# lowquark/uflow

Hardware: AMD Instinct MI355X
Metric: device-resident frame-CRC GiB/s (1500-B frames, validate: crc+valid per frame) (higher is better)
Workload: dtype u8

## Files before the change

### uflow_amd/csrc/frame_crc.hip

```cpp
#include "frame_crc_dev.hpp"

namespace ufc_dev {

struct RunAcc {
  uint32_t crc;
  uint32_t valid;
};

template <bool SEAL>
__device__ __forceinline__ void finish_set(const Lane& L, const KernelParams& p, const FrameDesc& d, const Chains& c,
                                           uint64_t set, int t, RunAcc& acc) {
  const uint32_t X0 = L.odd ? c.v2 : c.v0, X1 = L.odd ? c.v3 : c.v1;
  const uint32_t X2 = L.odd ? c.v0 : c.v2, X3 = L.odd ? c.v1 : c.v3;
  uint32_t lin = xor3(nib_mul<0>(L.lds, X0, L.K2), nib_mul<1>(L.lds, X1, L.K2), nib_mul<2>(L.lds, X2, L.K2)) ^
                 nib_mul<3>(L.lds, X3, L.K2);
  lin = row_xor16(lin);
  const uint32_t crc = ~lin;
  if (SEAL) {
    const uint64_t f = set * 4 + (uint64_t)L.grp;
    if (L.col == 15 && f < p.nframes && d.len >= 4u) {
      uint8_t* a = p.wbytes + d.start + d.n;
      if (((uintptr_t)a & 3u) == 0) {
        *as_global<g_u32w>((uint32_t*)a) = __builtin_bswap32(crc);
      } else {
// ... 132 lines not shown
    uint64_t r2;
    int t2;
    next_pos(r, tt, r2, t2);
    if (r2 != r) store_run<SEAL>(L, p, set_of(r, 0) * 4, acc);
  };

  FrameDesc d = desc_now(set_of(run, t));
  int parts = set_parts(d);
  while (set_slow(d, parts)) {
    slow_set<SEAL>(L, p, d, parts * JC, set_of(run, t), t, acc);
    after_set(run, t);
    next_pos(run, t, run, t);
    if (set_of(run, t) >= nsets) return;
    d = desc_now(set_of(run, t));
    parts = set_parts(d);
  }

  struct Cursor {
    uint64_t run;
    int t, part, parts;
    bool valid, slow;
    FrameDesc d;
  };
  uint64_t pre_a = 0, pre_b = 0;
  auto prefetch_offsets = [&](uint64_t r2, int t2) {
    if (VARLEN) {
      const uint64_t s2 = set_of(r2, t2);
      const uint64_t f = frame_index(s2 < nsets ? s2 : 0);
      pre_a = *as_global<g_u64>(p.offsets + f);
      pre_b = *as_global<g_u64>(p.offsets + f + 1);
    }
  };
  auto advance = [&](Cursor& c) {
    if (!c.valid || c.slow) {
      c.valid = false;
      return;
    }
    if (!SINGLE && c.part + 1 < c.parts) {
      c.part++;
      return;
    }
    uint64_t r2;
    int t2;
    next_pos(c.run, c.t, r2, t2);
    c.run = r2;
    c.t = t2;
    c.part = 0;
    if (set_of(r2, t2) >= nsets) {
      c.valid = false;
      return;
    }
    c.d = VARLEN ? make_desc(pre_a, pre_b - pre_a) : make_desc(frame_index(set_of(r2, t2)) * p.stride, p.frame_len);
    {
      uint64_t r3;
      int t3;
      next_pos(r2, t2, r3, t3);
      prefetch_offsets(r3, t3);
    }
    c.parts = set_parts(c.d);
    c.slow = set_slow(c.d, c.parts);
  };
  auto lane_base = [&](const Cursor& c) -> const uint8_t* { return p.bytes + c.d.start - c.d.pad + 16 * L.col; };

  Cursor C0{run, t, 0, parts, true, false, d};
  {
    uint64_t r2;
    int t2;
    next_pos(run, t, r2, t2);
    prefetch_offsets(r2, t2);
  }
  Cursor C1 = C0;
  advance(C1);
  Cursor C2 = C1;
  advance(C2);
  auto load_cursor = [&](const Cursor& c, ItemBuf<JC>& b) {
    const bool ok = c.valid && !c.slow;
    load_item<JC>(ok ? lane_base(c) : lane_base(C0), ok ? c.part : 0, b);
  };

  Chains c{0u, 0u, 0u, 0u, 0u};
  bool go_slow = false;
  uint64_t slow_run = 0;
  int slow_t = 0;
  auto step = [&](ItemBuf<JC>& cur, ItemBuf<JC>& nxt2) -> bool {
    {
      const bool ok = C2.valid && !C2.slow;
      const uint8_t* q = (ok ? lane_base(C2) : lane_base(C0)) + (int64_t)(ok ? C2.part : 0) * (JC * 256);
      const bool p0 = SINGLE || C0.part == 0;
      if (!p0) __builtin_assume(C0.part >= 1);
#pragma unroll
      for (int j = 0; j < JC; j++) {
        const u32x4 v = __builtin_nontemporal_load(as_global<g_u32x4>(q + 256 * j));
        nxt2.x[j] = make_uint4(v.x, v.y, v.z, v.w);
        __builtin_amdgcn_sched_barrier(0);
        if (p0)
          process_block<FREEZE>(L, C0.d, j, cur.x[j], c);
        else
          process_block<FREEZE>(L, C0.d, C0.part * JC + j, cur.x[j], c);
        __builtin_amdgcn_sched_barrier(0);
      }
    }
    if (SINGLE || C0.part + 1 == C0.parts) {
      finish_set<SEAL>(L, p, C0.d, c, set_of(C0.run, C0.t), C0.t, acc);
      after_set(C0.run, C0.t);
    }
    if (!C1.valid) return false;
    if (C1.slow) {
      go_slow = true;
      slow_run = C1.run;
      slow_t = C1.t;
      return false;
    }
    C0 = C1;
    C1 = C2;
    advance(C2);
    return true;
  };
  {
    ItemBuf<JC> X, Y, Z;
    load_cursor(C0, X);
    load_cursor(C1, Y);
    while (step(X, Z) && step(Y, X) && step(Z, Y)) {
    }
  }
  if (go_slow) {
    run = slow_run;
    t = slow_t;
    while (set_of(run, t) < nsets) {
      d = desc_now(set_of(run, t));
      parts = set_parts(d);
      slow_set<SEAL>(L, p, d, parts * JC, set_of(run, t), t, acc);
      after_set(run, t);
      next_pos(run, t, run, t);
    }
  }
}




constexpr int lean_loadv(int skip, int first, int mid, int last) { return skip | first << 1 | mid << 6 | last << 11; }
[[maybe_unused]] constexpr int kLoadvAllNT = lean_loadv(0, kFixAuxNT, kFixAuxNT, kFixAuxNT);
constexpr int kLoadvProduct = lean_loadv(0, 0, kFixAuxNT, kFixAuxNT);
template <int J, bool SEAL, int DEPTH, int SCHED, int WAVES, int LOADV = kLoadvProduct>
__global__ __launch_bounds__(WAVES * 64) void frame_crc_fixed_kernel(const KernelParams p) {
  static_assert(DEPTH >= 1 && DEPTH <= 3, "pipeline depth (4 spills at J = 6)");
  static_assert(DEPTH != 1 || SCHED != kSchedClaim, "depth 1: static schedules only");
  constexpr bool DYN = SCHED == kSchedClaim;
  constexpr bool ILV = SCHED == kSchedInterleave;
  constexpr uint32_t kInc = ILV ? (uint32_t)WAVES : 1u;
  __shared__ __attribute__((aligned(16))) char lds[kLdsBytes];
  const StageSet<WAVES * 64> sr = stage_load<WAVES * 64>(p);
  Lane L;
  init_lane(L, lds, p.G);

  const uint64_t stride = p.stride;
  const uint32_t len = (uint32_t)p.frame_len;
  const uint32_t n = len - 4u;
  const int pad = J * 256 - (int)len;
  const uint32_t nsets = (uint32_t)((p.nframes + 3) >> 2);
  const uint32_t nfull = (uint32_t)(p.nframes >> 2);
  const bool tail = (p.nframes & 3) != 0;
  const uint32_t wpb = WAVES;
  const uint32_t wid = __builtin_amdgcn_readfirstlane(threadIdx.x >> 6);
  const uint32_t w = blockIdx.x * wpb + wid;
  const uint32_t s_edge =
      p.front_ok ? 0u : (uint32_t)min(((uint64_t)pad + 4 * stride - 1) / (4 * stride), (uint64_t)nsets);
  const bool edge0 = s_edge == 1 && (p.nframes - 1) * stride + len >= 16;
  const uint32_t s_fast = edge0 ? 0u : s_edge;
  const uint32_t nfast = nfull - s_fast;
  uint32_t q_lo, q_end, q_cur, q_nx1, q_nx2;
  if (DYN || ILV) {
    q_lo = s_fast + (uint32_t)((uint64_t)nfast * blockIdx.x / gridDim.x);
    q_end = s_fast + (uint32_t)((uint64_t)nfast * (blockIdx.x + 1) / gridDim.x);
    q_cur = q_lo + wid;
    q_nx1 = q_lo + wpb + wid;
  } else {
    const uint32_t NW = gridDim.x * wpb;
    q_lo = s_fast + (uint32_t)((uint64_t)nfast * w / NW);
    q_end = s_fast + (uint32_t)((uint64_t)nfast * (w + 1) / NW);
    q_cur = q_lo;
    q_nx1 = q_lo + 1;
  }
  uint32_t* ctr = DYN ? p.ctr + blockIdx.x * kCtrWordsPerBlock : nullptr;
  auto claim_issue = [&]() -> uint32_t {
    uint32_t v = 0;
    if (L.lane == 0) v = __hip_atomic_fetch_add(ctr, 1u, __ATOMIC_RELAXED, __HIP_MEMORY_SCOPE_AGENT);
    return v;
  };
  auto claim_set = [&](uint32_t v) -> uint32_t {
    return q_lo + (DEPTH - 1) * wpb + __builtin_amdgcn_readfirstlane(v);
  };

  const int64_t lane_off = (int64_t)L.grp * (int64_t)stride + 16 * L.col - pad;
  uint32_t dm[4], pre[4];
#pragma unroll
  for (int b = 0; b < 4; b++) {
    const int o = 16 * L.col + 4 * b - pad;
    const uint32_t fz = fix_word(0u, o, L.G);
    const uint32_t f1 = fix_word(0xFFFFFFFFu, o, L.G);
    dm[b] = f1 & ~fz;
    pre[b] = fz;
  }
  uint32_t dm1, pre1;
  {
    const int o = 256 + 16 * L.col - pad;
    const uint32_t fz = fix_word(0u, o, L.G), f1 = fix_word(0xFFFFFFFFu, o, L.G);
    dm1 = f1 & ~fz;
    pre1 = fz;
  }
  const uint32_t tmask = (L.col == 15) ? 0u : 0xFFFFFFFFu;

  constexpr int RUNS = lean_runs(WAVES);
  uint32_t acc_crc = 0, acc_qv = 0;
  uint32_t hist_crc[RUNS], hist_qv[RUNS];
#pragma unroll
  for (int r = 0; r < RUNS; r++) hist_crc[r] = hist_qv[r] = 0;
  uint32_t t = 0, nhist = 0;
  auto write_trailer = [&](uint64_t f, uint32_t crc) {
    uint8_t* a = p.wbytes + f * stride + n;
    if (((uintptr_t)a & 3u) == 0) {
      *as_global<g_u32w>((uint32_t*)a) = __builtin_bswap32(crc);
    } else {
      g_u8w* wp = as_global<g_u8w>(a);
      wp[0] = (uint8_t)(crc >> 24);
      wp[1] = (uint8_t)(crc >> 16);
      wp[2] = (uint8_t)(crc >> 8);
      wp[3] = (uint8_t)crc;
    }
  };
  auto store_run = [&](int cnt, uint32_t crcs, uint32_t qv) {
    const uint64_t f = (uint64_t)(qv & 0x7FFFFFFFu) * 4 + (uint64_t)L.grp;
    if (L.col < cnt && f < p.nframes) {
      if (p.crc_out) *as_global<g_u32w>(p.crc_out + f) = crcs;
      if (!SEAL && p.valid_out) *as_global<g_u8w>(p.valid_out + f) = (uint8_t)(qv >> 31);
      if (SEAL) write_trailer(f, crcs);
    }
  };
  auto store_all = [&]() {
    if (t > 0) store_run((int)t, acc_crc, acc_qv);
#pragma unroll
    for (int r = 0; r < RUNS; r++)
      if ((uint32_t)r < nhist) store_run(kSetsPerRun, hist_crc[r], hist_qv[r]);
  };
  auto finish = [&](uint32_t q, const Chains& c, bool may_overflow) {
    const uint32_t crc = ~group_lin(L, c);
    const uint32_t tr = (uint32_t)__builtin_amdgcn_update_dpp(0, (int)c.tr, 0x15F, 0xF, 0xF, false);
    const uint32_t ok = (len >= 5u && __builtin_bswap32(tr) == crc) ? 1u : 0u;
    acc_crc = (L.col == (int)t) ? crc : acc_crc;
    acc_qv = (L.col == (int)t) ? (q | (ok << 31)) : acc_qv;
    if (++t == kSetsPerRun) {
      if (may_overflow && nhist == RUNS) {
        t = 0;
        store_all();
        __builtin_amdgcn_s_waitcnt(0x0F70);
        nhist = 0;
      }
#pragma unroll
      for (int r = RUNS - 1; r > 0; r--) {
        hist_crc[r] = hist_crc[r - 1];
        hist_qv[r] = hist_qv[r - 1];
      }
      hist_crc[0] = acc_crc;
      hist_qv[0] = acc_qv;
      nhist++;
      t = 0;
    }
  };
  auto compute_block = [&](uint32_t q, int j, uint4 x, Chains& c) {
    {
      if (j == J - 1) {
        c.tr = x.w;
        x.w &= tmask;
      }
      if (j == 0) {
        c.v0 = (x.x & dm[0]) | pre[0];
        c.v1 = (x.y & dm[1]) | pre[1];
        c.v2 = (x.z & dm[2]) | pre[2];
        c.v3 = (x.w & dm[3]) | pre[3];
      } else {
        if (j == 1) x.x = (x.x & dm1) | pre1;
        c.v0 = chain_step(L.lds, c.v0, L.K, x.x);
        c.v1 = chain_step(L.lds, c.v1, L.K, x.y);
        c.v2 = chain_step(L.lds, c.v2, L.K, x.z);
        c.v3 = chain_step(L.lds, c.v3, L.K, x.w);
      }
    }
  };
  auto compute = [&](uint32_t q, const ItemBuf<J>& b, Chains& c) {
#pragma unroll
    for (int j = 0; j < J; j++) compute_block(q, j, b.x[j], c);
  };
  const uint32_t voff = (uint32_t)(lane_off + 512);
  auto set_base = [&](uint32_t q) -> const uint8_t* {
    return p.bytes + (uint64_t)(q < q_end ? q : nfull - 1) * 4 * stride - 512;
  };
  auto load_edge0 = [&](ItemBuf<J>& b) {
    const int64_t room = (int64_t)min(p.nframes - 1, (uint64_t)3);
    const int64_t over = (int64_t)L.grp > room ? (int64_t)L.grp - room : 0;
    const int64_t off0 = lane_off - over * (int64_t)stride;
#pragma unroll
    for (int j = 0; j < J; j++) {
      const int64_t off = off0 + 256 * j;
      uint4 v = load_frame16<true>(p.bytes + (off < 0 ? 0 : off));
      if (off < 0) {
        const int64_t d = -off;
        uint64_t lo = (uint64_t)v.x | ((uint64_t)v.y << 32), hi = (uint64_t)v.z | ((uint64_t)v.w << 32);
        if (d >= 16) {
          lo = hi = 0;
        } else if (d >= 8) {
          hi = lo << (8 * (d - 8));
          lo = 0;
        } else {
          hi = (hi << (8 * d)) | (lo >> (64 - 8 * d));
          lo = lo << (8 * d);
        }
        v = make_uint4((uint32_t)lo, (uint32_t)(lo >> 32), (uint32_t)hi, (uint32_t)(hi >> 32));
      }
      b.x[j] = v;
    }
  };
  const uint32_t voff_b0 = ((LOADV & 1) && 16 * L.col + 16 <= pad - 4) ? kFixRecords : voff;
  auto load = [&](uint32_t q, ItemBuf<J>& b) {
    constexpr int kAuxFirst = (LOADV >> 1) & 31, kAuxMid = (LOADV >> 6) & 31, kAuxLast = (LOADV >> 11) & 31;
    const __amdgpu_buffer_rsrc_t rs =
        __builtin_amdgcn_make_buffer_rsrc((void*)set_base(q), 0, (int)kFixRecords, kFixRsrcWord3);
#pragma unroll
    for (int j = 0; j < J; j++) {
      const uint32_t o = (j == 0 ? voff_b0 : voff) + 256u * j;
      u32x4 v;
      if (j == 0)
        v = __builtin_amdgcn_raw_buffer_load_b128(rs, (int)o, 0, kAuxFirst);
      else if (j == J - 1)
        v = __builtin_amdgcn_raw_buffer_load_b128(rs, (int)o, 0, kAuxLast);
      else
        v = __builtin_amdgcn_raw_buffer_load_b128(rs, (int)o, 0, kAuxMid);
      b.x[j] = make_uint4(v.x, v.y, v.z, v.w);
    }
  };
  auto load_tail = [&](ItemBuf<J>& b) {
    const int64_t room = (int64_t)(p.nframes - 1 - 4 * (uint64_t)nfull);
    const int64_t over = (int64_t)L.grp > room ? (int64_t)L.grp - room : 0;
    load_set<J>(p.bytes + (uint64_t)nfull * 4 * stride - 512, voff - (uint32_t)(over * (int64_t)stride), b);
  };

  ItemBuf<J> A, B, C;
  uint32_t cX = 0, cY = 0, cZ = 0;
  if (DYN) {
    cY = claim_issue();
    cZ = claim_issue();
  }
  if (edge0 && q_cur == 0)
    load_edge0(A);
  else
    load(q_cur, A);
  if (DEPTH == 3) load(q_nx1, B);
  stage_store<WAVES * 64>(sr, lds);
  q_nx2 = (DEPTH == 3 && !DYN) ? q_cur + 2 * kInc : 0;

  if (w == 0 && s_fast > 0) {
#pragma unroll 1
    for (uint32_t e = 0; e < s_fast; e++) {
      FrameDesc d = make_desc(min((uint64_t)e * 4 + (uint64_t)L.grp, p.nframes - 1) * stride, len);
      Chains ce{0u, 0u, 0u, 0u, 0u};
#pragma unroll 1
      for (int blk = 0; blk < J; blk++) {
        uint32_t wv[4];
#pragma unroll
        for (int b = 0; b < 4; b++) {
          const int o = 256 * blk + 16 * L.col + 4 * b - d.pad;
          uint32_t a = 0;
#pragma unroll 1
          for (int k = 0; k < 4; k++) {
            const int ob = o + k;
            if (ob >= 0 && ob < (int)d.len) a |= (uint32_t)*as_global<g_u8>(p.bytes + d.start + (uint64_t)ob) << (8 * k);
          }
          wv[b] = a;
        }
        process_block<false>(L, d, blk, make_uint4(wv[0], wv[1], wv[2], wv[3]), ce);
      }
      const uint32_t crc = ~group_lin(L, ce);
      const uint32_t ok = (len >= 5u && __builtin_bswap32(ce.tr) == crc) ? 1u : 0u;
      const uint64_t f = (uint64_t)e * 4 + (uint64_t)L.grp;
      if (L.col == 15 && f < p.nframes) {
        if (p.crc_out) *as_global<g_u32w>(p.crc_out + f) = crc;
        if (!SEAL && p.valid_out) *as_global<g_u8w>(p.valid_out + f) = (uint8_t)ok;
        if (SEAL) write_trailer(f, crc);
      }
    }
    __builtin_amdgcn_s_waitcnt(0x0F70);
  }


  Chains c{0u, 0u, 0u, 0u, 0u};
  auto step = [&](ItemBuf<J>& cur, ItemBuf<J>& fill, uint32_t& c_issue, uint32_t& c_read) {
    uint32_t q_load;
    if (DYN) {
      q_load = claim_set(c_read);
      c_issue = claim_issue();
    } else {
      q_load = (DEPTH == 3) ? q_nx2 : q_nx1;
    }
    load(q_load, fill);
    __builtin_amdgcn_sched_barrier(0);
    if (q_cur < q_end) {
      compute(q_cur, cur, c);
      finish(q_cur, c, DYN);
    }
    __builtin_amdgcn_sched_barrier(0);
    if (DEPTH == 3) {
      q_cur = q_nx1;
      q_nx1 = q_load;
      q_nx2 = q_load + kInc;
    } else {
      q_cur = q_load;
      q_nx1 = q_load + kInc;
    }
  };
  if (DEPTH == 1) {
    while (q_cur < q_end) {
      compute(q_cur, A, c);
      finish(q_cur, c, false);
      q_cur += kInc;
      load(q_cur, A);
    }
  } else if (DEPTH == 2 && !DYN) {
    while (q_cur < q_end) {
      step(A, B, cX, cY);
      step(B, A, cY, cZ);
    }
  } else if (DEPTH == 2) {
    while (q_cur < q_end) {
      step(A, B, cX, cY);
      step(B, A, cY, cZ);
      step(A, B, cZ, cX);
      step(B, A, cX, cY);
      step(A, B, cY, cZ);
      step(B, A, cZ, cX);
    }
  } else {
    while (q_cur < q_end) {
      step(A, C, cX, cY);
      step(B, A, cY, cZ);
      step(C, B, cZ, cX);
    }
  }
  if (tail && blockIdx.x == gridDim.x - 1 && wid == wpb - 1) {
    ItemBuf<J> T;
    load_tail(T);
    compute(nfull, T, c);
    const uint32_t crc = ~group_lin(L, c);
    const uint32_t tr = (uint32_t)__builtin_amdgcn_update_dpp(0, (int)c.tr, 0x15F, 0xF, 0xF, false);
    const uint32_t ok = (len >= 5u && __builtin_bswap32(tr) == crc) ? 1u : 0u;
    const uint64_t f = (uint64_t)nfull * 4 + (uint64_t)L.grp;
    if (L.col == 0 && f < p.nframes) {
      if (p.crc_out) *as_global<g_u32w>(p.crc_out + f) = crc;
      if (!SEAL && p.valid_out) *as_global<g_u8w>(p.valid_out + f) = (uint8_t)ok;
      if (SEAL) write_trailer(f, crc);
    }
  }
  if (DYN) {
    store_all();
  } else {
    uint32_t blo = q_lo, bhi = q_end;
    if (!ILV) {
      const uint64_t NW = (uint64_t)gridDim.x * wpb;
      blo = s_fast + (uint32_t)((uint64_t)nfast * (blockIdx.x * wpb) / NW);
      bhi = s_fast + (uint32_t)((uint64_t)nfast * ((blockIdx.x + 1) * wpb) / NW);
    }
    const uint32_t nfr = 4 * (bhi - blo);
    uint32_t* lcrc = (uint32_t*)lds;
    uint8_t* lval = (uint8_t*)lds + 4 * nfr;
    __builtin_amdgcn_fence(__ATOMIC_RELEASE, "workgroup", "local");
    __builtin_amdgcn_s_barrier();
    __builtin_amdgcn_fence(__ATOMIC_ACQUIRE, "workgroup", "local");
    auto stage = [&](int cnt, uint32_t crcs, uint32_t qv) {
      if (L.col < cnt) {
        const uint32_t q = qv & 0x7FFFFFFFu;
        const uint32_t pos = (q - blo) * 4 + (uint32_t)L.grp;
        lcrc[pos] = crcs;
        lval[pos] = (uint8_t)(qv >> 31);
      }
    };
    if (t > 0) stage((int)t, acc_crc, acc_qv);
#pragma unroll
    for (int r = 0; r < RUNS; r++)
      if ((uint32_t)r < nhist) stage(kSetsPerRun, hist_crc[r], hist_qv[r]);
    __builtin_amdgcn_fence(__ATOMIC_RELEASE, "workgroup", "local");
    __builtin_amdgcn_s_barrier();
    __builtin_amdgcn_fence(__ATOMIC_ACQUIRE, "workgroup", "local");
    const uint64_t f0 = (uint64_t)blo * 4;
    if (p.crc_out)
      for (uint32_t i = threadIdx.x; i < nfr; i += WAVES * 64) *as_global<g_u32w>(p.crc_out + f0 + i) = lcrc[i];
    if (SEAL) {
      for (uint32_t i = threadIdx.x; i < nfr; i += WAVES * 64) {
        const uint32_t v = __builtin_bswap32(lcrc[i]);
        uint8_t* a = p.wbytes + (f0 + i) * stride + n;
        if (((uintptr_t)a & 3u) == 0) {
          __builtin_nontemporal_store(v, as_global<g_u32w>((uint32_t*)a));
        } else {
          g_u8w* wp = as_global<g_u8w>(a);
          __builtin_nontemporal_store((uint8_t)v, wp);
          __builtin_nontemporal_store((uint8_t)(v >> 8), wp + 1);
          __builtin_nontemporal_store((uint8_t)(v >> 16), wp + 2);
          __builtin_nontemporal_store((uint8_t)(v >> 24), wp + 3);
        }
      }
    }
    if (!SEAL && p.valid_out) {
      if ((((uintptr_t)(p.valid_out + f0)) & 3u) == 0) {
        for (uint32_t i = threadIdx.x; i < nfr / 4; i += WAVES * 64)
          *as_global<g_u32w>((uint32_t*)(p.valid_out + f0) + i) = ((const uint32_t*)lval)[i];
      } else {
        for (uint32_t i = threadIdx.x; i < nfr; i += WAVES * 64) *as_global<g_u8w>(p.valid_out + f0 + i) = lval[i];
      }
    }
  }

  if (DYN) {
    __builtin_amdgcn_s_waitcnt(0x0F70);
    uint32_t done = 0;
    if (L.lane == 0) done = __hip_atomic_fetch_add(ctr + 1, 1u, __ATOMIC_RELAXED, __HIP_MEMORY_SCOPE_AGENT);
    if (__builtin_amdgcn_readfirstlane(done) == wpb - 1 && L.lane == 0) {
      __hip_atomic_store(ctr, 0u, __ATOMIC_RELAXED, __HIP_MEMORY_SCOPE_AGENT);
      __hip_atomic_store(ctr + 1, 0u, __ATOMIC_RELAXED, __HIP_MEMORY_SCOPE_AGENT);
    }
  }
}

#define UFC_INST_FIXED(J)                                                                                  \
  template __global__ void frame_crc_fixed_kernel<J, false, 2, kSchedInterleave, 8>(const KernelParams); \
  template __global__ void frame_crc_fixed_kernel<J, true, 2, kSchedInterleave, 8>(const KernelParams);
UFC_INST_FIXED(1) UFC_INST_FIXED(2) UFC_INST_FIXED(3) UFC_INST_FIXED(4) UFC_INST_FIXED(5) UFC_INST_FIXED(6)


const void* fixed_kernel_symbol(int J, bool seal, int depth, int sched, int waves) {
  if (depth == 2 && sched == kSchedInterleave && waves == 8) {
    switch (J) {
#define UFC_PICK_FIXED(JJ)                                                                          \
  case JJ:                                                                                          \
    return seal ? (const void*)frame_crc_fixed_kernel<JJ, true, 2, kSchedInterleave, 8>          \
                : (const void*)frame_crc_fixed_kernel<JJ, false, 2, kSchedInterleave, 8>;
      UFC_PICK_FIXED(1) UFC_PICK_FIXED(2) UFC_PICK_FIXED(3) UFC_PICK_FIXED(4) UFC_PICK_FIXED(5) UFC_PICK_FIXED(6)
#undef UFC_PICK_FIXED
      default: return nullptr;
    }
  }
  return nullptr;
}

#define UFC_INST_MODES(JC)                                                                          \
  template __global__ void frame_crc_kernel<JC, 0>(const KernelParams);                             \
  template __global__ void frame_crc_kernel<JC, kModeSeal>(const KernelParams);                     \
  template __global__ void frame_crc_kernel<JC, kModeFreeze>(const KernelParams);                   \
  template __global__ void frame_crc_kernel<JC, kModeFreeze | kModeSeal>(const KernelParams);       \
  template __global__ void frame_crc_kernel<JC, kModeVarlen>(const KernelParams);                   \
  template __global__ void frame_crc_kernel<JC, kModeVarlen | kModeSeal>(const KernelParams);

#define UFC_CONFIGS(X) X(1) X(2) X(3) X(4) X(5) X(6)

UFC_CONFIGS(UFC_INST_MODES)


const void* kernel_symbol(int jc, int mode) {
#define UFC_PICK(JC)                                                                                   \
  if (jc == JC) {                                                                                      \
    switch (mode) {                                                                                    \
      case 0: return (const void*)frame_crc_kernel<JC, 0>;                                            \
      case kModeSeal: return (const void*)frame_crc_kernel<JC, kModeSeal>;                            \
      case kModeFreeze: return (const void*)frame_crc_kernel<JC, kModeFreeze>;                        \
      case kModeFreeze | kModeSeal: return (const void*)frame_crc_kernel<JC, kModeFreeze | kModeSeal>; \
      case kModeVarlen: return (const void*)frame_crc_kernel<JC, kModeVarlen>;                        \
      case kModeVarlen | kModeSeal: return (const void*)frame_crc_kernel<JC, kModeVarlen | kModeSeal>; \
      default: break;                                                                                  \
    }                                                                                                  \
  }
  UFC_CONFIGS(UFC_PICK)
#undef UFC_PICK
  return nullptr;
}

bool config_available(int jc) { return jc >= 1 && jc <= 6; }

namespace {
__global__ __launch_bounds__(256) void seal_scatter_kernel(uint8_t* bytes, uint64_t stride, uint64_t n_off,
                                                           uint64_t nframes, const uint32_t* crc) {
  for (uint64_t i = (uint64_t)blockIdx.x * 256 + threadIdx.x; i < nframes; i += (uint64_t)gridDim.x * 256) {
    const uint32_t v = __builtin_bswap32(crc[i]);
    uint8_t* a = bytes + i * stride + n_off;
    if (((uintptr_t)a & 3u) == 0) {
      __builtin_nontemporal_store(v, (uint32_t*)a);
    } else {
      __builtin_nontemporal_store((uint8_t)v, a);
      __builtin_nontemporal_store((uint8_t)(v >> 8), a + 1);
      __builtin_nontemporal_store((uint8_t)(v >> 16), a + 2);
      __builtin_nontemporal_store((uint8_t)(v >> 24), a + 3);
    }
  }
}
}

int seal_scatter(uint8_t* bytes, uint64_t stride, uint64_t frame_len, uint64_t nframes, const uint32_t* crc,
                 void* stream) {
  if (nframes == 0) return 0;
  const uint64_t blocks = std::min<uint64_t>((nframes + 255) / 256, 1u << 20);
  hipLaunchKernelGGL(seal_scatter_kernel, dim3((unsigned)blocks), dim3(256), 0, (hipStream_t)stream, bytes, stride,
                     frame_len - 4, nframes, crc);
  return (int)hipGetLastError();
}

}
```

### uflow_amd/csrc/frame_crc_kernels.hpp

```cpp
#pragma once
#include <cstdint>

namespace ufc_dev {

constexpr int kModeVarlen = 1;
constexpr int kModeSeal = 2;
constexpr int kModeFreeze = 4;

constexpr int kBlockThreads = 1024;
constexpr int kLdsBytes = 131072 + 32768;

struct KernelParams {
  const uint8_t* bytes;
  uint8_t* wbytes;
  const uint64_t* offsets;
  uint64_t stride;
  uint64_t frame_len;
  uint64_t nframes;
  uint32_t* crc_out;
  uint8_t* valid_out;
  const uint32_t* chain_tab;
  const uint32_t* nib_img;
  uint32_t G;
  uint32_t* ctr;
  uint32_t front_ok;
  uint32_t* defer_list;
  uint32_t* defer_counts;
};

const void* kernel_symbol(int jc, int mode);
bool config_available(int jc);
constexpr int kLeanDepthDefault = 2;
constexpr int kLeanRuns = 8;
constexpr int lean_runs(int waves) { return waves == 8 ? 32 : kLeanRuns; }
constexpr int kLeanWavesDefault = 8;
constexpr int kSchedRange = 0;
constexpr int kSchedClaim = 1;
constexpr int kSchedInterleave = 2;
constexpr int kLeanSchedDefault = kSchedInterleave;
const void* fixed_kernel_symbol(int J, bool seal, int depth, int sched, int waves);
constexpr int kRunFrames = 64;
const void* varlen8_kernel_symbol(bool seal, bool pairs);
int varlen8_waves();
const void* long8_kernel_symbol(bool seal, bool pairs);
int slots_to_pairs(const uint32_t* d_lens, uint64_t stride, uint64_t n, uint64_t* d_pairs, void* stream);
int seal_scatter(uint8_t* bytes, uint64_t stride, uint64_t frame_len, uint64_t nframes, const uint32_t* crc,
                 void* stream);
int read_stream(const uint8_t* bytes, uint64_t nbytes, uint32_t* sink, int ncu, void* stream);
constexpr int kCtrWordsPerBlock = 32;

}
```

### uflow_amd/csrc/ufc_api.cpp

```cpp
#include <hip/hip_runtime.h>

#include <algorithm>
#include <atomic>
#include <cstdio>
#include <cstdlib>
#include <cstring>
#include <mutex>
#include <new>
#include <vector>

#include "../../include/uflow_frame_codec.h"
#include "../../include/uflow_frame_crc.h"
#include "crc_math.hpp"
#include "frame_build.hpp"
#include "frame_crc_kernels.hpp"
#include "frame_pack.hpp"
#include "frame_parse.hpp"
#include "frame_queue.hpp"
#include "frame_window.hpp"
#include "flush_ctl.hpp"
#include "packet_emit.hpp"
#include "packet_receive.hpp"
#include "resend.hpp"
#include "route.hpp"
#include "send_rate.hpp"
#include "ufc_internal.hpp"

struct ufc_ctx {
  int device = -1;
  int ncu = 0;
  uint32_t* d_chain = nullptr;
  uint32_t* d_nib = nullptr;
  uint32_t* d_chain128 = nullptr;
  uint32_t* d_nib32 = nullptr;
  uint32_t G = 0;
  int last_hip_error = 0;
  std::atomic<int> stalled_comms{0};
  uint8_t* d_stage = nullptr;
  size_t d_stage_cap = 0;
  uint64_t* d_off = nullptr;
  size_t d_off_cap = 0;
  uint32_t* d_crc = nullptr;
  uint8_t* d_valid = nullptr;
  size_t d_out_cap = 0;
  uint64_t* h_off_pinned = nullptr;
  hipStream_t streams[2] = {nullptr, nullptr};
  uint32_t* d_ctr = nullptr;
  std::atomic<uint32_t> ctr_seq{0};
  int opt[UFC_OPT_COUNT_] = {};
  struct Scratch {
    int kind;
    hipStream_t stream;
    void* p;
    size_t cap;
  };
  std::mutex scratch_mu;
  std::vector<Scratch> scratch;
};

constexpr uint32_t kCtrSlots = 64;

namespace {

enum ScratchKind {
  kScratchParse = 0,
  kScratchAsyncSlots = 2,
  kScratchSealCrc = 3,
  kScratchDeferList = 4,
  kScratchDeferCounts = 5,
  kScratchBuild = 6,
  kScratchPack = 7,
  kScratchEmit = 8,
  kScratchReceive = 9,
  kScratchWindow = 10,
  kScratchFlushAcks = 11,
  kScratchFlushSync = 12,
  kScratchRoute = 13
};

hipError_t stream_scratch(ufc_ctx* ctx, int kind, hipStream_t stream, size_t need, void** out, bool* fresh = nullptr) {
  if (fresh) *fresh = false;
  std::lock_guard<std::mutex> lk(ctx->scratch_mu);
  ufc_ctx::Scratch* sc = nullptr;
  for (auto& x : ctx->scratch)
    if (x.kind == kind && x.stream == stream) sc = &x;
  if (!sc) {
    ctx->scratch.push_back({kind, stream, nullptr, 0});
    sc = &ctx->scratch.back();
  }
  if (sc->cap < need) {
    hipError_t e;
    if (sc->p) {
      if ((e = hipStreamSynchronize(stream)) != hipSuccess) return e;
      (void)hipFree(sc->p);
      sc->p = nullptr;
      sc->cap = 0;
    }
    if ((e = hipMalloc(&sc->p, need)) != hipSuccess) return e;
    sc->cap = need;
    if (fresh) *fresh = true;
  }
  *out = sc->p;
  return hipSuccess;
}

struct DeviceGuard {
  int prev = -1;
  explicit DeviceGuard(int dev) {
    if (hipGetDevice(&prev) != hipSuccess) prev = -1;
    if (prev != dev) (void)hipSetDevice(dev);
  }
  ~DeviceGuard() {
    int cur = -1;
    if (prev >= 0 && hipGetDevice(&cur) == hipSuccess && cur != prev) (void)hipSetDevice(prev);
  }
};

int hip_fail(ufc_ctx* ctx, hipError_t e) {
  if (ctx) ctx->last_hip_error = (int)e;
  return UFC_ERR_HIP;
}

struct Config {
  int jc;
};

int launch(ufc_ctx* ctx, Config cfg, int mode, ufc_dev::KernelParams& kp, hipStream_t stream) {
  const void* fn = ufc_dev::kernel_symbol(cfg.jc, mode);
  if (!fn) return UFC_ERR_INVALID_ARG;
  const uint64_t nsets = (kp.nframes + 3) / 4;
  const uint64_t nruns = (nsets + 15) / 16;
  const uint64_t waves_per_block = ufc_dev::kBlockThreads / 64;
  uint64_t blocks = (nruns + waves_per_block - 1) / waves_per_block;
  if (blocks > (uint64_t)ctx->ncu) blocks = (uint64_t)ctx->ncu;
  if (blocks < 1) blocks = 1;
  kp.chain_tab = ctx->d_chain;
  kp.nib_img = ctx->d_nib;
  kp.G = ctx->G;
  void* args[] = {&kp};
  hipError_t e = hipLaunchKernel(fn, dim3((unsigned)blocks), dim3(ufc_dev::kBlockThreads), args, 0, stream);
  if (e != hipSuccess) return hip_fail(ctx, e);
  return UFC_OK;
}

int lean_fixed_blocks(const ufc_ctx* ctx, uint64_t frame_len, uint64_t stride, uint64_t n) {
  if (frame_len < 4) return 0;
  const uint64_t J = (frame_len + 4 + 255) / 256;
  if (J > 6 || stride >= (1ull << 28)) return 0;
  const uint64_t pad = 256 * J - frame_len;
  const uint64_t s_edge = (pad + 4 * stride - 1) / (4 * stride);
  if (n / 4 <= s_edge) return 0;
  if (ctx->opt[UFC_OPT_FIXED_KERNEL] == UFC_FIXED_GENERIC || ctx->opt[UFC_OPT_GENERIC_JC] != 0) return 0;
  return (int)J;
}

int launch_lean_fixed(ufc_ctx* ctx, int J, bool seal, ufc_dev::KernelParams& kp, hipStream_t stream,
                      bool front_ok = false) {
  const int depth = ufc_dev::kLeanDepthDefault, waves = ufc_dev::kLeanWavesDefault;
  const int sched = ufc_dev::kLeanSchedDefault;
  const void* fn = ufc_dev::fixed_kernel_symbol(J, seal, depth, sched, waves);
  if (!fn) return UFC_ERR_INVALID_ARG;
  kp.chain_tab = ctx->d_chain;
  kp.nib_img = ctx->d_nib;
  kp.G = ctx->G;
  const uint64_t waves_per_block = (uint64_t)waves;
  const uint64_t chunk = (uint64_t)ctx->ncu * waves_per_block * (16 * ufc_dev::lean_runs(waves) - 1) * 4;
  const uint64_t total = kp.nframes;
  for (uint64_t f0 = 0, step = 0; f0 < total; f0 += step) {
    ufc_dev::KernelParams c = kp;
    c.nframes = std::min(chunk, total - f0);
    if (total - f0 - c.nframes > 0 && total - f0 - c.nframes < 4) c.nframes -= 4;
    step = c.nframes;
    c.bytes = kp.bytes + f0 * kp.stride;
    if (kp.wbytes) c.wbytes = kp.wbytes + f0 * kp.stride;
    if (kp.crc_out) c.crc_out = kp.crc_out + f0;
    if (kp.valid_out) c.valid_out = kp.valid_out + f0;
    c.front_ok = (f0 > 0 || front_ok) ? 1u : 0u;
    const uint32_t slot = ctx->ctr_seq.fetch_add(1) % kCtrSlots;
    c.ctr = ctx->d_ctr + (size_t)slot * ctx->ncu * ufc_dev::kCtrWordsPerBlock;
    const uint64_t nsets = (c.nframes + 3) / 4;
    uint64_t blocks = (nsets + waves_per_block - 1) / waves_per_block;
    if (blocks > (uint64_t)ctx->ncu) blocks = (uint64_t)ctx->ncu;
    if (blocks < 1) blocks = 1;
    void* args[] = {&c};
    hipError_t e = hipLaunchKernel(fn, dim3((unsigned)blocks), dim3((unsigned)(waves * 64)), args, 0, stream);
    if (e != hipSuccess) return hip_fail(ctx, e);
  }
  return UFC_OK;
}


int launch_varlen8(ufc_ctx* ctx, bool seal, bool pairs, ufc_dev::KernelParams& kp, hipStream_t stream) {
  const void* fn = ufc_dev::varlen8_kernel_symbol(seal, pairs);
  const void* fn_long = ufc_dev::long8_kernel_symbol(seal, pairs);
  if (!fn || !fn_long) return UFC_ERR_INVALID_ARG;
  const int waves = ufc_dev::varlen8_waves();
  kp.chain_tab = ctx->d_chain128;
  kp.nib_img = ctx->d_nib32;
  kp.G = ctx->G;
  const uint64_t chunk = (uint64_t)1 << 29;
  const uint64_t total = kp.nframes;
  void* list = nullptr;
  void* counts = nullptr;
  bool fresh = false;
  hipError_t e;
  const uint64_t nmax = std::min(chunk, total);
  if ((e = stream_scratch(ctx, kScratchDeferList, stream, (size_t)(nmax + 64) * 4, &list)) != hipSuccess ||
      (e = stream_scratch(ctx, kScratchDeferCounts, stream, (size_t)ctx->ncu * 4, &counts, &fresh)) != hipSuccess)
    return hip_fail(ctx, e);
  if (fresh && (e = hipMemsetAsync(counts, 0, (size_t)ctx->ncu * 4, stream)) != hipSuccess) return hip_fail(ctx, e);
  for (uint64_t f0 = 0; f0 < total; f0 += chunk) {
    ufc_dev::KernelParams c = kp;
    c.nframes = std::min(chunk, total - f0);
    c.offsets = kp.offsets + (pairs ? 2 * f0 : f0);
    if (kp.crc_out) c.crc_out = kp.crc_out + f0;
    if (kp.valid_out) c.valid_out = kp.valid_out + f0;
    c.defer_list = (uint32_t*)list;
    c.defer_counts = (uint32_t*)counts;
    const uint64_t nruns = (c.nframes + 63) / 64;
    uint64_t blocks = (nruns + waves - 1) / waves;
    if (blocks > (uint64_t)ctx->ncu) blocks = (uint64_t)ctx->ncu;
    if (blocks < 1) blocks = 1;
    void* args[] = {&c};
    if ((e = hipLaunchKernel(fn, dim3((unsigned)blocks), dim3((unsigned)(waves * 64)), args, 0, stream)) != hipSuccess)
      return hip_fail(ctx, e);
    uint32_t nb = (uint32_t)blocks;
    void* args_long[] = {&c, &nb};
    if ((e = hipLaunchKernel(fn_long, dim3((unsigned)blocks), dim3((unsigned)(waves * 64)), args_long, 0, stream)) !=
        hipSuccess)
      return hip_fail(ctx, e);
  }
  return UFC_OK;
}

Config fixed_config(const ufc_ctx* ctx, uint64_t frame_len, int* freeze) {
  const uint64_t n = frame_len >= 4 ? frame_len - 4 : frame_len;
  const uint64_t J = (n + 8 + 255) / 256;
  Config c;
  const int jc = ctx->opt[UFC_OPT_GENERIC_JC];
  c.jc = ufc_dev::config_available(jc) ? jc : (J <= 6 ? (int)J : 6);
  *freeze = ((uint64_t)c.jc == J) ? 0 : ufc_dev::kModeFreeze;
  return c;
}

Config varlen_config(const ufc_ctx* ctx) {
  const int jc = ctx->opt[UFC_OPT_GENERIC_JC];
  return Config{ufc_dev::config_available(jc) ? jc : 3};
}

int launch_varlen_any(ufc_ctx* ctx, bool seal, bool pairs, ufc_dev::KernelParams& kp, hipStream_t stream) {
  if (ctx->opt[UFC_OPT_VARLEN_KERNEL] == UFC_VARLEN_GENERIC && !pairs)
    return launch(ctx, varlen_config(ctx), ufc_dev::kModeVarlen | (seal ? ufc_dev::kModeSeal : 0), kp, stream);
  return launch_varlen8(ctx, seal, pairs, kp, stream);
}

using ufc_internal::kMaxFrameLen;

hipError_t grow_staging(ufc_ctx* ctx, size_t stage_bytes, size_t off_entries, size_t out_frames) {
  hipError_t e;
  if (ctx->d_stage_cap < stage_bytes) {
    if (ctx->d_stage) (void)hipFree(ctx->d_stage);
    ctx->d_stage = nullptr;
    ctx->d_stage_cap = 0;
    if ((e = hipMalloc(&ctx->d_stage, stage_bytes)) != hipSuccess) return e;
    ctx->d_stage_cap = stage_bytes;
  }
  if (ctx->d_off_cap < off_entries) {
    if (ctx->d_off) (void)hipFree(ctx->d_off);
    if (ctx->h_off_pinned) (void)hipHostFree(ctx->h_off_pinned);
    ctx->d_off = nullptr;
    ctx->h_off_pinned = nullptr;
    ctx->d_off_cap = 0;
    if ((e = hipMalloc(&ctx->d_off, off_entries * 8)) != hipSuccess) return e;
    if ((e = hipHostMalloc(&ctx->h_off_pinned, off_entries * 8, hipHostMallocDefault)) != hipSuccess) return e;
    ctx->d_off_cap = off_entries;
  }
  if (ctx->d_out_cap < out_frames) {
    if (ctx->d_crc) (void)hipFree(ctx->d_crc);
    if (ctx->d_valid) (void)hipFree(ctx->d_valid);
    ctx->d_crc = nullptr;
    ctx->d_valid = nullptr;
    ctx->d_out_cap = 0;
    if ((e = hipMalloc(&ctx->d_crc, out_frames * 4)) != hipSuccess) return e;
    if ((e = hipMalloc(&ctx->d_valid, out_frames)) != hipSuccess) return e;
    ctx->d_out_cap = out_frames;
  }
  return hipSuccess;
}

}

hipError_t ufc_dev::ScratchSource::get(size_t bytes, char** out) const {
  return stream_scratch(ctx, kind, stream, bytes, (void**)out);
}

extern "C" {

uint32_t ufc_crc32_compute(const uint8_t* data, size_t len) {
  if (!data) return 0;
  return ufc::host_extend(0u, data, len);
}

uint32_t ufc_crc32_extend(uint32_t initial_crc, const uint8_t* data, size_t len) {
  if (!data) return initial_crc;
  return ufc::host_extend(initial_crc, data, len);
}

int ufc_frame_validate(const uint8_t* frame, size_t len) {
  if (!frame || len < 5) return 0;
  const uint32_t c = ufc::host_extend(0u, frame, len - 4);
  const uint8_t* t = frame + len - 4;
  const uint32_t rx = ((uint32_t)t[0] << 24) | ((uint32_t)t[1] << 16) | ((uint32_t)t[2] << 8) | (uint32_t)t[3];
  return c == rx ? 1 : 0;
}

int ufc_frame_seal(uint8_t* frame, size_t len) {
  if (!frame || len < 4) return UFC_ERR_INVALID_ARG;
  const uint32_t c = ufc::host_extend(0u, frame, len - 4);
  uint8_t* t = frame + len - 4;
  t[0] = (uint8_t)(c >> 24);
  t[1] = (uint8_t)(c >> 16);
  t[2] = (uint8_t)(c >> 8);
  t[3] = (uint8_t)c;
  return UFC_OK;
}

int ufc_device_count(void) {
  int n = 0;
  if (hipGetDeviceCount(&n) != hipSuccess) return 0;
  return n;
}

const char* ufc_error_string(int code) {
  switch (code) {
    case UFC_OK: return "ok";
    case UFC_ERR_INVALID_ARG: return "invalid argument";
// ... 777 lines not shown
```

Baseline: 6120.

## Precompute lean partition geometry on host and issue first loads before LDS init

Moves the per-block work-range and edge computation (64-bit divides) into a host-side helper passed through kernel params as quotient/remainder. The first frame-set loads, plus the next one in the depth-2 static schedule, are issued before lane/LDS initialization. The old per-lane edge0 gather path is replaced by a clamped buffer load with an in-register shift fix. The depth-2 loop is peeled so the first set is computed outside the ping-pong loop. This targets kernel prologue latency, at the cost of a reordered params struct and new edge-case handling.

After: 6109. No clear change (-0.2%).

```diff
diff --git a/uflow_amd/csrc/frame_crc.hip b/uflow_amd/csrc/frame_crc.hip
--- a/uflow_amd/csrc/frame_crc.hip
+++ b/uflow_amd/csrc/frame_crc.hip
@@ -308,33 +308,32 @@
   __shared__ __attribute__((aligned(16))) char lds[kLdsBytes];
   const StageSet<WAVES * 64> sr = stage_load<WAVES * 64>(p);
   Lane L;
-  init_lane(L, lds, p.G);
+  L.lane = threadIdx.x & 63;
+  L.col = L.lane & 15;
+  L.grp = L.lane >> 4;
 
   const uint64_t stride = p.stride;
   const uint32_t len = (uint32_t)p.frame_len;
   const uint32_t n = len - 4u;
   const int pad = J * 256 - (int)len;
-  const uint32_t nsets = (uint32_t)((p.nframes + 3) >> 2);
   const uint32_t nfull = (uint32_t)(p.nframes >> 2);
   const bool tail = (p.nframes & 3) != 0;
   const uint32_t wpb = WAVES;
   const uint32_t wid = __builtin_amdgcn_readfirstlane(threadIdx.x >> 6);
   const uint32_t w = blockIdx.x * wpb + wid;
-  const uint32_t s_edge =
-      p.front_ok ? 0u : (uint32_t)min(((uint64_t)pad + 4 * stride - 1) / (4 * stride), (uint64_t)nsets);
-  const bool edge0 = s_edge == 1 && (p.nframes - 1) * stride + len >= 16;
-  const uint32_t s_fast = edge0 ? 0u : s_edge;
-  const uint32_t nfast = nfull - s_fast;
+  const bool front_ok = (p.lean_flags & kLeanFrontOk) != 0, edge0 = (p.lean_flags & kLeanEdge0) != 0;
+  const uint32_t s_fast = p.s_fast;
+  const uint32_t b_lo = lean_range_lo(s_fast, p.rq, p.rr, blockIdx.x);
+  const uint32_t b_end = lean_range_lo(s_fast, p.rq, p.rr, blockIdx.x + 1);
   uint32_t q_lo, q_end, q_cur, q_nx1, q_nx2;
   if (DYN || ILV) {
-    q_lo = s_fast + (uint32_t)((uint64_t)nfast * blockIdx.x / gridDim.x);
-    q_end = s_fast + (uint32_t)((uint64_t)nfast * (blockIdx.x + 1) / gridDim.x);
+    q_lo = b_lo;
+    q_end = b_end;
     q_cur = q_lo + wid;
     q_nx1 = q_lo + wpb + wid;
   } else {
-    const uint32_t NW = gridDim.x * wpb;
-    q_lo = s_fast + (uint32_t)((uint64_t)nfast * w / NW);
-    q_end = s_fast + (uint32_t)((uint64_t)nfast * (w + 1) / NW);
+    q_lo = b_lo + (uint32_t)((uint64_t)(b_end - b_lo) * wid / wpb);
+    q_end = b_lo + (uint32_t)((uint64_t)(b_end - b_lo) * (wid + 1) / wpb);
     q_cur = q_lo;
     q_nx1 = q_lo + 1;
   }
@@ -348,7 +347,72 @@
     return q_lo + (DEPTH - 1) * wpb + __builtin_amdgcn_readfirstlane(v);
   };
 
-  const int64_t lane_off = (int64_t)L.grp * (int64_t)stride + 16 * L.col - pad;
+  const int32_t lane_off = (int32_t)((uint32_t)L.grp * (uint32_t)stride) + 16 * L.col - pad;
+  const uint32_t voff = (uint32_t)(lane_off + 512);
+  auto set_base = [&](uint32_t q) -> const uint8_t* {
+    return p.bytes + (uint64_t)(q < q_end ? q : nfull - 1) * 4 * stride - 512;
+  };
+  const uint32_t voff_b0 = ((LOADV & 1) && 16 * L.col + 16 <= pad - 4) ? kFixRecords : voff;
+  constexpr int kAuxFirst = (LOADV >> 1) & 31, kAuxMid = (LOADV >> 6) & 31, kAuxLast = (LOADV >> 11) & 31;
+  auto load_block = [&](__amdgpu_buffer_rsrc_t rs, int j, uint32_t o) -> uint4 {
+    u32x4 v;
+    if (j == 0)
+      v = __builtin_amdgcn_raw_buffer_load_b128(rs, (int)o, 0, kAuxFirst);
+    else if (j == J - 1)
+      v = __builtin_amdgcn_raw_buffer_load_b128(rs, (int)o, 0, kAuxLast);
+    else
+      v = __builtin_amdgcn_raw_buffer_load_b128(rs, (int)o, 0, kAuxMid);
+    return make_uint4(v.x, v.y, v.z, v.w);
+  };
+  auto load = [&](uint32_t q, ItemBuf<J>& b) {
+    const __amdgpu_buffer_rsrc_t rs =
+        __builtin_amdgcn_make_buffer_rsrc((void*)set_base(q), 0, (int)kFixRecords, kFixRsrcWord3);
+#pragma unroll
+    for (int j = 0; j < J; j++) b.x[j] = load_block(rs, j, (j == 0 ? voff_b0 : voff) + 256u * j);
+  };
+  auto load_first = [&](uint32_t q, ItemBuf<J>& b) {
+    const uint64_t boff = (uint64_t)(q < q_end ? q : nfull - 1) * 4 * stride;
+    const uint32_t adj = front_ok ? 512u : (uint32_t)min(boff, (uint64_t)512);
+    const __amdgpu_buffer_rsrc_t rs =
+        __builtin_amdgcn_make_buffer_rsrc((void*)(p.bytes + boff - adj), 0, (int)kFixRecords, kFixRsrcWord3);
+#pragma unroll
+    for (int j = 0; j < J; j++) b.x[j] = load_block(rs, j, (uint32_t)max(lane_off + (int32_t)adj + 256 * j, 0));
+  };
+  auto fix_edge0 = [&](ItemBuf<J>& b) {
+#pragma unroll
+    for (int j = 0; j < J; j++) {
+      const int off = lane_off + 256 * j;
+      if (off < 0) {
+        const int d = -off;
+        const uint4 v = b.x[j];
+        uint64_t lo = (uint64_t)v.x | ((uint64_t)v.y << 32), hi = (uint64_t)v.z | ((uint64_t)v.w << 32);
+        if (d >= 16) {
+          lo = hi = 0;
+        } else if (d >= 8) {
+          hi = lo << (8 * (d - 8));
+          lo = 0;
+        } else if (d > 0) {
+          hi = (hi << (8 * d)) | (lo >> (64 - 8 * d));
+          lo = lo << (8 * d);
+        }
+        b.x[j] = make_uint4((uint32_t)lo, (uint32_t)(lo >> 32), (uint32_t)hi, (uint32_t)(hi >> 32));
+      }
+    }
+  };
+
+  constexpr bool PEEL = DEPTH == 2 && !DYN;
+  ItemBuf<J> A, B, C;
+  uint32_t cX = 0, cY = 0, cZ = 0;
+  if (DYN) {
+    cY = claim_issue();
+    cZ = claim_issue();
+  }
+  const bool fix0 = edge0 && q_cur == 0 && q_cur < q_end;
+  load_first(q_cur, A);
+  if (DEPTH == 3 || PEEL) load(q_nx1, B);
+  __builtin_amdgcn_sched_barrier(0);
+
+  init_lane(L, lds, p.G);
   uint32_t dm[4], pre[4];
 #pragma unroll
   for (int b = 0; b < 4; b++) {
@@ -447,70 +511,12 @@
 #pragma unroll
     for (int j = 0; j < J; j++) compute_block(q, j, b.x[j], c);
   };
-  const uint32_t voff = (uint32_t)(lane_off + 512);
-  auto set_base = [&](uint32_t q) -> const uint8_t* {
-    return p.bytes + (uint64_t)(q < q_end ? q : nfull - 1) * 4 * stride - 512;
-  };
-  auto load_edge0 = [&](ItemBuf<J>& b) {
-    const int64_t room = (int64_t)min(p.nframes - 1, (uint64_t)3);
-    const int64_t over = (int64_t)L.grp > room ? (int64_t)L.grp - room : 0;
-    const int64_t off0 = lane_off - over * (int64_t)stride;
-#pragma unroll
-    for (int j = 0; j < J; j++) {
-      const int64_t off = off0 + 256 * j;
-      uint4 v = load_frame16<true>(p.bytes + (off < 0 ? 0 : off));
-      if (off < 0) {
-        const int64_t d = -off;
-        uint64_t lo = (uint64_t)v.x | ((uint64_t)v.y << 32), hi = (uint64_t)v.z | ((uint64_t)v.w << 32);
-        if (d >= 16) {
-          lo = hi = 0;
-        } else if (d >= 8) {
-          hi = lo << (8 * (d - 8));
-          lo = 0;
-        } else {
-          hi = (hi << (8 * d)) | (lo >> (64 - 8 * d));
-          lo = lo << (8 * d);
-        }
-        v = make_uint4((uint32_t)lo, (uint32_t)(lo >> 32), (uint32_t)hi, (uint32_t)(hi >> 32));
-      }
-      b.x[j] = v;
-    }
-  };
-  const uint32_t voff_b0 = ((LOADV & 1) && 16 * L.col + 16 <= pad - 4) ? kFixRecords : voff;
-  auto load = [&](uint32_t q, ItemBuf<J>& b) {
-    constexpr int kAuxFirst = (LOADV >> 1) & 31, kAuxMid = (LOADV >> 6) & 31, kAuxLast = (LOADV >> 11) & 31;
-    const __amdgpu_buffer_rsrc_t rs =
-        __builtin_amdgcn_make_buffer_rsrc((void*)set_base(q), 0, (int)kFixRecords, kFixRsrcWord3);
-#pragma unroll
-    for (int j = 0; j < J; j++) {
-      const uint32_t o = (j == 0 ? voff_b0 : voff) + 256u * j;
-      u32x4 v;
-      if (j == 0)
-        v = __builtin_amdgcn_raw_buffer_load_b128(rs, (int)o, 0, kAuxFirst);
-      else if (j == J - 1)
-        v = __builtin_amdgcn_raw_buffer_load_b128(rs, (int)o, 0, kAuxLast);
-      else
-        v = __builtin_amdgcn_raw_buffer_load_b128(rs, (int)o, 0, kAuxMid);
-      b.x[j] = make_uint4(v.x, v.y, v.z, v.w);
-    }
-  };
   auto load_tail = [&](ItemBuf<J>& b) {
     const int64_t room = (int64_t)(p.nframes - 1 - 4 * (uint64_t)nfull);
     const int64_t over = (int64_t)L.grp > room ? (int64_t)L.grp - room : 0;
     load_set<J>(p.bytes + (uint64_t)nfull * 4 * stride - 512, voff - (uint32_t)(over * (int64_t)stride), b);
   };
 
-  ItemBuf<J> A, B, C;
-  uint32_t cX = 0, cY = 0, cZ = 0;
-  if (DYN) {
-    cY = claim_issue();
-    cZ = claim_issue();
-  }
-  if (edge0 && q_cur == 0)
-    load_edge0(A);
-  else
-    load(q_cur, A);
-  if (DEPTH == 3) load(q_nx1, B);
   stage_store<WAVES * 64>(sr, lds);
   q_nx2 = (DEPTH == 3 && !DYN) ? q_cur + 2 * kInc : 0;
 
@@ -547,6 +553,7 @@
     __builtin_amdgcn_s_waitcnt(0x0F70);
   }
 
+  if (fix0) fix_edge0(A);
 
   Chains c{0u, 0u, 0u, 0u, 0u};
   auto step = [&](ItemBuf<J>& cur, ItemBuf<J>& fill, uint32_t& c_issue, uint32_t& c_read) {
@@ -580,10 +587,17 @@
       q_cur += kInc;
       load(q_cur, A);
     }
-  } else if (DEPTH == 2 && !DYN) {
+  } else if (PEEL) {
+    if (q_cur < q_end) {
+      compute(q_cur, A, c);
+      finish(q_cur, c, false);
+    }
+    __builtin_amdgcn_sched_barrier(0);
+    q_cur = q_nx1;
+    q_nx1 += kInc;
     while (q_cur < q_end) {
+      step(B, A, cY, cZ);
       step(A, B, cX, cY);
-      step(B, A, cY, cZ);
     }
   } else if (DEPTH == 2) {
     while (q_cur < q_end) {
@@ -618,12 +632,7 @@
   if (DYN) {
     store_all();
   } else {
-    uint32_t blo = q_lo, bhi = q_end;
-    if (!ILV) {
-      const uint64_t NW = (uint64_t)gridDim.x * wpb;
-      blo = s_fast + (uint32_t)((uint64_t)nfast * (blockIdx.x * wpb) / NW);
-      bhi = s_fast + (uint32_t)((uint64_t)nfast * ((blockIdx.x + 1) * wpb) / NW);
-    }
+    const uint32_t blo = b_lo, bhi = b_end;
     const uint32_t nfr = 4 * (bhi - blo);
     uint32_t* lcrc = (uint32_t*)lds;
     uint8_t* lval = (uint8_t*)lds + 4 * nfr;
diff --git a/uflow_amd/csrc/frame_crc_kernels.hpp b/uflow_amd/csrc/frame_crc_kernels.hpp
--- a/uflow_amd/csrc/frame_crc_kernels.hpp
+++ b/uflow_amd/csrc/frame_crc_kernels.hpp
@@ -10,23 +10,46 @@
 constexpr int kBlockThreads = 1024;
 constexpr int kLdsBytes = 131072 + 32768;
 
+constexpr uint32_t kLeanFrontOk = 1;
+constexpr uint32_t kLeanEdge0 = 2;
+
 struct KernelParams {
   const uint8_t* bytes;
-  uint8_t* wbytes;
-  const uint64_t* offsets;
   uint64_t stride;
   uint64_t frame_len;
   uint64_t nframes;
-  uint32_t* crc_out;
-  uint8_t* valid_out;
+  uint32_t rq, rr;
+  uint32_t s_fast;
+  uint32_t lean_flags;
   const uint32_t* chain_tab;
   const uint32_t* nib_img;
   uint32_t G;
+  uint32_t* crc_out;
+  uint8_t* valid_out;
+  uint8_t* wbytes;
   uint32_t* ctr;
-  uint32_t front_ok;
+  const uint64_t* offsets;
   uint32_t* defer_list;
   uint32_t* defer_counts;
 };
+
+struct LeanGeom {
+  uint32_t rq, rr, s_fast, flags;
+};
+constexpr LeanGeom lean_geometry(uint64_t frame_len, uint64_t stride, uint64_t nframes, bool front_ok, uint32_t grid) {
+  const uint64_t J = (frame_len + 4 + 255) / 256, pad = 256 * J - frame_len;
+  const uint64_t nsets = (nframes + 3) >> 2, nfull = nframes >> 2;
+  const uint64_t e = (pad + 4 * stride - 1) / (4 * stride);
+  const uint64_t s_edge = front_ok ? 0 : (e < nsets ? e : nsets);
+  const bool edge0 = s_edge == 1 && (nframes - 1) * stride + frame_len >= 16;
+  const uint64_t s_fast = edge0 ? 0 : s_edge;
+  const uint64_t nfast = nfull > s_fast ? nfull - s_fast : 0;
+  return LeanGeom{(uint32_t)(nfast / grid), (uint32_t)(nfast % grid), (uint32_t)s_fast,
+                  (front_ok ? kLeanFrontOk : 0u) | (edge0 ? kLeanEdge0 : 0u)};
+}
+constexpr uint32_t lean_range_lo(uint32_t s_fast, uint32_t rq, uint32_t rr, uint32_t b) {
+  return s_fast + rq * b + (b < rr ? b : rr);
+}
 
 const void* kernel_symbol(int jc, int mode);
 bool config_available(int jc);
diff --git a/uflow_amd/csrc/ufc_api.cpp b/uflow_amd/csrc/ufc_api.cpp
--- a/uflow_amd/csrc/ufc_api.cpp
+++ b/uflow_amd/csrc/ufc_api.cpp
@@ -175,13 +175,18 @@
     if (kp.wbytes) c.wbytes = kp.wbytes + f0 * kp.stride;
     if (kp.crc_out) c.crc_out = kp.crc_out + f0;
     if (kp.valid_out) c.valid_out = kp.valid_out + f0;
-    c.front_ok = (f0 > 0 || front_ok) ? 1u : 0u;
     const uint32_t slot = ctx->ctr_seq.fetch_add(1) % kCtrSlots;
     c.ctr = ctx->d_ctr + (size_t)slot * ctx->ncu * ufc_dev::kCtrWordsPerBlock;
     const uint64_t nsets = (c.nframes + 3) / 4;
     uint64_t blocks = (nsets + waves_per_block - 1) / waves_per_block;
     if (blocks > (uint64_t)ctx->ncu) blocks = (uint64_t)ctx->ncu;
     if (blocks < 1) blocks = 1;
+    const ufc_dev::LeanGeom g =
+        ufc_dev::lean_geometry(kp.frame_len, kp.stride, c.nframes, f0 > 0 || front_ok, (uint32_t)blocks);
+    c.rq = g.rq;
+    c.rr = g.rr;
+    c.s_fast = g.s_fast;
+    c.lean_flags = g.flags;
     void* args[] = {&c};
     hipError_t e = hipLaunchKernel(fn, dim3((unsigned)blocks), dim3((unsigned)(waves * 64)), args, 0, stream);
     if (e != hipSuccess) return hip_fail(ctx, e);
```
